# AcherStyx/SSD-Object-Detection

Hardware: AMD Instinct MI355X
Metric: images/sec SSD300 train step, batch 64 (higher is better)
Workload: dtype bf16; 1 GPU; BASELINE configs[2]: SSD300 full train step (anchor match+encode, image normalisation, conv fwd, loss, conv bwd, per-variable clip (64 variables) + Adam), per-GPU batch 64, 80 classes, synthetic COCO-shaped boxes; per_gpu_batch=64, global_batch=64, parallelism=single

## Files before the change

include/ssd_hip.h:

```cpp
#ifndef SSD_HIP_H
#define SSD_HIP_H

#include <stddef.h>
#include <stdint.h>

#ifdef __cplusplus
extern "C" {
#endif

typedef enum {
    SSD_OK = 0,
    SSD_ERR_ASSERT = -1,
    SSD_ERR_VALUE = -2,
    SSD_ERR_WORKSPACE = -3,
    SSD_ERR_LAUNCH = -4,
    SSD_ERR_UNSUPPORTED = -5
} ssd_status;

typedef enum { SSD_F32 = 0, SSD_BF16 = 1 } ssd_dtype;

int ssd_hip_abi_version(void);
const char* ssd_status_string(int status);

int ssd_priors_count(const int* grid_hw, int levels, const int* ratio_off);
// ... 189 lines not shown
int ssd_heads_bwd_data_sparse_levels(const ssd_head_grads* hg, const ssd_head_layers* hl, int B, unsigned level_mask,
                                     void* ws, size_t ws_bytes, void* stream);
size_t ssd_heads_bwd_weight_sparse_workspace_bytes(int B, const ssd_head_grads* hg, const ssd_head_layers* hl);
int ssd_heads_bwd_weight_sparse(const ssd_head_grads* hg, const ssd_head_layers* hl, int B, void* ws, size_t ws_bytes,
                                void* stream);

int ssd_head_grad_pack(const void* dloc, const void* dconf, void* out, int B, int hw, int per_cell, int classes,
                       int npad, int anchors_total, int level_off, void* stream);

int ssd_opt_block_elems(void);
int ssd_grad_clip_scales(const float* grad, long long n, const int32_t* tensor_block_off, int ntensors, float clip,
                         double* partial, float* scale, float* norms, void* stream);
int ssd_grad_apply_scale(float* grad, long long n, const int32_t* block_tensor, const float* scale, void* stream);
int ssd_grad_accumulate(float* acc, const float* grad, long long n, const int32_t* block_tensor, const float* scale,
                        int first, void* stream);
int ssd_adam_step(float* param, const float* grad, float* m, float* v, void* param_bf16, long long n,
                  const int32_t* block_tensor, const float* scale, float grad_scale, float lr_t, float beta1,
                  float beta2, float eps, void* stream);
int ssd_sgd_step(float* param, const float* grad, void* param_bf16, long long n, const int32_t* block_tensor,
                 const float* scale, float grad_scale, float lr, void* stream);

enum ssd_conv_plan {
    SSD_PLAN_KERNEL_MASK = 0xff,
    SSD_PLAN_C64B = 1, SSD_PLAN_P32_64, SSD_PLAN_P32_128, SSD_PLAN_8PH,
    SSD_PLAN_DMA_256_256, SSD_PLAN_DMA_256_128, SSD_PLAN_DMA_256_64, SSD_PLAN_DMA_128_64, SSD_PLAN_DMA_128_128,
    SSD_PLAN_CONV0_FWD, SSD_PLAN_P512, SSD_PLAN_PW,
    SSD_PLAN_WG_FIRST = 32, SSD_PLAN_WG_PATCH_16x16, SSD_PLAN_WG_PATCH_6x40, SSD_PLAN_WG_PATCH_10x24, SSD_PLAN_WG_TILE,
    SSD_PLAN_WG_GENERIC,
    SSD_PLAN_F_FLAT = 0x100,
    SSD_PLAN_F_ROWFLAT = 0x200,
    SSD_PLAN_F_SPLITK = 0x400,
    SSD_PLAN_F_POOL_FUSED = 0x800,
    SSD_PLAN_F_S2 = 0x1000,
    SSD_PLAN_F_REDUCE_WIDE = 0x2000
};
int ssd_conv2d_fwd_plan(int B, int H, int W, int Cin, int Cout, int ksize, int stride, int pad_t, int pad_l, int Ho, int Wo,
                        int pool, size_t ws_bytes);
int ssd_conv2d_head_fwd_plan(int B, int H, int W, int Cin, int per_cell, int classes, size_t ws_bytes);
int ssd_conv2d_bwd_data_plan(int B, int H, int W, int Cin, int Cout_pad, int ksize, int stride, int pad_t, int pad_l, int Ho,
                             int Wo, int accumulate, size_t ws_bytes);
int ssd_conv2d_bwd_weight_plan(int B, int H, int W, int Cin, int Cout, int ldy, int ksize, int stride, int pad_t, int pad_l,
                               int Ho, int Wo);
const char* ssd_conv_plan_name(int plan);
int ssd_conv2d_fwd_workgroups(int B, int H, int W, int Cin, int Cout, int ksize, int stride, int pad_t, int pad_l, int Ho,
                              int Wo, int pool, size_t ws_bytes);
int ssd_conv2d_bwd_data_workgroups(int B, int H, int W, int Cin, int Cout_pad, int ksize, int stride, int pad_t, int pad_l,
                                   int Ho, int Wo, int accumulate, size_t ws_bytes);

int ssd_dev_knob(const char* name, int value);

int ssd_dev_mfma_calibration_workgroups(void);
double ssd_dev_mfma_calibration_flops(int iters);
int ssd_dev_mfma_calibration(int iters, void* stamps, void* sink, void* stream);

#ifdef __cplusplus
}
#endif
#endif
```

ssd-object-detection_amd/_lib.py:

```python
import ctypes
import os

HERE = os.path.dirname(os.path.abspath(__file__))
LIB_PATH = os.path.join(HERE, os.environ.get("SSD_HIP_LIB", "libssd_hip.so"))

SSD_OK, SSD_ERR_ASSERT, SSD_ERR_VALUE, SSD_ERR_WORKSPACE, SSD_ERR_LAUNCH, SSD_ERR_UNSUPPORTED = 0, -1, -2, -3, -4, -5
SSD_MAX_LEVELS = 8

_c_int_p = ctypes.POINTER(ctypes.c_int)
_c_double_p = ctypes.POINTER(ctypes.c_double)
VP = ctypes.c_void_p


class PriorGrid(ctypes.Structure):
    _fields_ = [("levels", ctypes.c_int),
                ("grid_h", ctypes.c_int * SSD_MAX_LEVELS),
                ("grid_w", ctypes.c_int * SSD_MAX_LEVELS),
                ("per_cell", ctypes.c_int * SSD_MAX_LEVELS),
                ("verified", ctypes.c_int)]


class HeadGrads(ctypes.Structure):
    _fields_ = [("levels", ctypes.c_int),
                ("hw", ctypes.c_int * SSD_MAX_LEVELS),
# ... 88 lines not shown
    "ssd_conv2d_bwd_data_wgrad_first": (ctypes.c_int, [VP] * 6 + [ctypes.c_int] * 3 + [VP, ctypes.c_size_t, VP]),
    "ssd_conv2d_bwd_weight_workspace_bytes": (ctypes.c_size_t, [ctypes.c_int] * 7),
    "ssd_conv2d_bwd_weight": (ctypes.c_int, [VP, VP, VP, VP] + [ctypes.c_int] * 12 + [VP, ctypes.c_size_t, VP]),
    "ssd_weight_transpose": (ctypes.c_int, [VP, VP, ctypes.c_int, ctypes.c_int, ctypes.c_int, ctypes.c_int, VP]),
    "ssd_cast_bf16": (ctypes.c_int, [VP, VP, ctypes.c_longlong, VP]),
    "ssd_image_prep": (ctypes.c_int, [VP, VP, ctypes.c_int, ctypes.c_int, ctypes.c_int, ctypes.c_int, VP]),
    "ssd_image_resize_prep": (ctypes.c_int, [VP, VP, VP, VP, ctypes.c_int, ctypes.c_int, ctypes.c_int, VP]),
    "ssd_box_prep": (ctypes.c_int, [VP, VP, VP, VP, ctypes.c_int, ctypes.c_int, VP]),
    "ssd_augment_plan": (ctypes.c_int, [VP, VP, VP, VP, ctypes.c_int, ctypes.c_int, ctypes.c_int, ctypes.c_uint64,
                                        ctypes.c_int64, VP, VP, VP, VP, VP]),
    "ssd_augment_image": (ctypes.c_int, [VP, ctypes.c_int, VP, VP, VP, VP, ctypes.c_int, ctypes.c_int, ctypes.c_int, VP]),
    "ssd_maxpool2x2_fwd": (ctypes.c_int, [VP, VP] + [ctypes.c_int] * 6 + [VP]),
    "ssd_maxpool2x2_bwd": (ctypes.c_int, [VP, VP, VP, VP] + [ctypes.c_int] * 6 + [VP]),
    "ssd_weight_transpose_batched": (ctypes.c_int, [VP, ctypes.c_int, ctypes.c_int, VP]),
    "ssd_maxpool2x2_fwd_argmax": (ctypes.c_int, [VP, VP, VP] + [ctypes.c_int] * 6 + [VP]),
    "ssd_maxpool2x2_bwd_argmax": (ctypes.c_int, [VP, VP, VP] + [ctypes.c_int] * 6 + [VP]),
    "ssd_head_grad_pack": (ctypes.c_int, [VP, VP, VP] + [ctypes.c_int] * 7 + [VP]),
    "ssd_opt_block_elems": (ctypes.c_int, []),
    "ssd_grad_clip_scales": (ctypes.c_int, [VP, ctypes.c_longlong, VP, ctypes.c_int, ctypes.c_float, VP, VP, VP, VP]),
    "ssd_grad_apply_scale": (ctypes.c_int, [VP, ctypes.c_longlong, VP, VP, VP]),
    "ssd_grad_accumulate": (ctypes.c_int, [VP, VP, ctypes.c_longlong, VP, VP, ctypes.c_int, VP]),
    "ssd_adam_step": (ctypes.c_int, [VP, VP, VP, VP, VP, ctypes.c_longlong, VP, VP] + [ctypes.c_float] * 5 + [VP]),
    "ssd_sgd_step": (ctypes.c_int, [VP, VP, VP, ctypes.c_longlong, VP, VP, ctypes.c_float, ctypes.c_float, VP]),
    "ssd_dev_knob": (ctypes.c_int, [ctypes.c_char_p, ctypes.c_int]),
    "ssd_dev_mfma_calibration_workgroups": (ctypes.c_int, []),
    "ssd_dev_mfma_calibration_flops": (ctypes.c_double, [ctypes.c_int]),
    "ssd_dev_mfma_calibration": (ctypes.c_int, [ctypes.c_int, VP, VP, VP]),
    "ssd_conv2d_fwd_plan": (ctypes.c_int, [ctypes.c_int] * 12 + [ctypes.c_size_t]),
    "ssd_conv2d_head_fwd_plan": (ctypes.c_int, [ctypes.c_int] * 6 + [ctypes.c_size_t]),
    "ssd_conv2d_bwd_data_plan": (ctypes.c_int, [ctypes.c_int] * 12 + [ctypes.c_size_t]),
    "ssd_conv2d_fwd_workgroups": (ctypes.c_int, [ctypes.c_int] * 12 + [ctypes.c_size_t]),
    "ssd_conv2d_bwd_data_workgroups": (ctypes.c_int, [ctypes.c_int] * 12 + [ctypes.c_size_t]),
    "ssd_conv2d_bwd_weight_plan": (ctypes.c_int, [ctypes.c_int] * 12),
    "ssd_conv_plan_name": (ctypes.c_char_p, [ctypes.c_int]),
    "ssd_loss_workspace_bytes": (ctypes.c_size_t, [ctypes.c_int, ctypes.c_int, ctypes.c_int]),
    "ssd_loss_heads_workspace_bytes": (ctypes.c_size_t, [ctypes.c_int, ctypes.c_int, ctypes.c_int]),
    "ssd_loss_fwd_bwd_heads": (ctypes.c_int, [VP, VP, ctypes.c_int, VP, VP, VP, ctypes.c_int, ctypes.c_int, ctypes.c_int,
                                              ctypes.c_float, VP, _HG, VP, ctypes.c_size_t, ctypes.c_int, VP]),
    "ssd_heads_bwd_data_sparse_workspace_bytes": (ctypes.c_size_t, [ctypes.c_int, _HL]),
    "ssd_heads_bwd_data_sparse": (ctypes.c_int, [_HG, _HL, ctypes.c_int, VP, ctypes.c_size_t, VP]),
    "ssd_heads_bwd_data_sparse_levels": (ctypes.c_int, [_HG, _HL, ctypes.c_int, ctypes.c_uint, VP, ctypes.c_size_t, VP]),
    "ssd_heads_bwd_weight_sparse_workspace_bytes": (ctypes.c_size_t, [ctypes.c_int, _HG, _HL]),
    "ssd_heads_bwd_weight_sparse": (ctypes.c_int, [_HG, _HL, ctypes.c_int, VP, ctypes.c_size_t, VP]),
    "ssd_loss_fwd_bwd": (ctypes.c_int, [VP, VP, ctypes.c_int, VP, VP, VP, ctypes.c_int, ctypes.c_int, ctypes.c_int,
                                        ctypes.c_float, VP, VP, VP, VP, ctypes.c_size_t, VP]),
}

_lib = None


def lib():
    global _lib
    if _lib is None:
        if not os.path.exists(LIB_PATH):
            raise RuntimeError(
                "libssd_hip.so is missing (%s): build it with `python ssd-object-detection_amd/build.py` "
                "or __graft_entry__.build(); there is no CPU fallback." % LIB_PATH)
        try:
            import torch
        except ImportError:
            pass
        L = ctypes.CDLL(LIB_PATH)
        for name, (res, args) in _SIGNATURES.items():
            fn = getattr(L, name)
            fn.restype = res
            fn.argtypes = args
# ... 14 lines not shown
```

ssd-object-detection_amd/csrc/conv.hip:

```cpp
#include <atomic>
#include <climits>
#include <cstdint>
#include <cstring>
#include <type_traits>
#include "common.h"
#include <hip/hip_bf16.h>
#include <stdlib.h>

#include "conv_common.h"
namespace {

template <int EPI>
__global__ void k_igemm_finalize(ConvGeom g, Epilogue ep) {
    const int n4 = (g.N + 3) >> 2;
    const long long idx = (long long)blockIdx.x * blockDim.x + threadIdx.x;
    if (idx >= (long long)g.M * n4) return;
    const int m = (int)(idx / n4), n = (int)(idx - (long long)m * n4) * 4;
    const bool full = n + 3 < g.N;
    float v[4] = {0.f, 0.f, 0.f, 0.f};
    if (full && !(g.N & 3)) {
        for (int z = 0; z < ep.ksplit; ++z) {
            const float4 t = *reinterpret_cast<const float4*>(ep.slab + ((long long)z * g.M + m) * g.N + n);
            v[0] += t.x; v[1] += t.y; v[2] += t.z; v[3] += t.w;
        }
// ... 1678 lines not shown
                for (int c = 0; c < 4; ++c)
                    acc[a][c] = __builtin_amdgcn_mfma_f32_16x16x32_bf16(fa[a], fb[c], acc[a][c], 0, 0, 0);
                if constexpr (BIAS) accb[a] = __builtin_amdgcn_mfma_f32_16x16x32_bf16(fa[a], ones, accb[a], 0, 0, 0);
            }
        }
    };
    if (do_bias) run(std::true_type{}); else run(std::false_type{});

    float* out = slab_w + (long long)split * g.N * ktot;
#pragma unroll
    for (int a = 0; a < 8; ++a)
#pragma unroll
        for (int c = 0; c < 4; ++c) {
            const int col = col0 + wave_n * 64 + c * 16 + (lane & 15);
            if (col >= ktot) continue;
#pragma unroll
            for (int j = 0; j < 4; ++j) {
                const int co = co0 + wave_m * 128 + a * 16 + (lane >> 4) * 4 + j;
                if (co < g.N) out[(long long)co * ktot + col] = acc[a][c][j];
            }
        }
    if (do_bias && (lane & 15) == 0) {
        float* ob = slab_b + (long long)split * g.N;
#pragma unroll
        for (int a = 0; a < 8; ++a)
#pragma unroll
            for (int j = 0; j < 4; ++j) {
                const int co = co0 + wave_m * 128 + a * 16 + (lane >> 4) * 4 + j;
                if (co < g.N) ob[co] = accb[a][j];
            }
    }
}

template <int BH, int BW8>
struct WpGeom {
    static constexpr int BW = BW8 * 8;
    static constexpr int PW = BW + 2, PH = BH + 2;
    static constexpr int PPIX = PW * PH;
    static constexpr int P_INSTR = (PPIX * 8 + 63) / 64;
    static constexpr int P_BYTES = P_INSTR * 1024;
    static constexpr int NPG = (BH / 2) * BW8;
    static constexpr int KS = (NPG + 1) / 2;
    static constexpr int DY_PIX = KS * 32;
    static constexpr int DY_BYTES = DY_PIX * 128;
    static constexpr int DY_INSTR = DY_PIX / 8;
    static constexpr int BUF = DY_BYTES + P_BYTES;
    static_assert(BH % 2 == 0 && DY_INSTR % 8 == 0, "block shape");
};

__device__ __forceinline__ int wp_key(int px) { return (px >> 1) & 3; }

template <int BH, int BW8>
__global__ __launch_bounds__(512) void k_conv3x3_wgrad_patch(const bf16_raw* __restrict__ x, const bf16_raw* __restrict__ dy,
                                                             float* __restrict__ slab_w, float* __restrict__ slab_b,
                                                             ConvGeom g, int tiles_x, int tiles_y, int tiles_per_split,
                                                             int nsplit, int cout, int single_buf, int xg) {
    using G = WpGeom<BH, BW8>;
    extern __shared__ __attribute__((aligned(16))) char smem[];

    const int tid = threadIdx.x, lane = tid & 63;
    const int wave = __builtin_amdgcn_readfirstlane(tid >> 6);
    const int ct = wave & 3, role = wave >> 2;
    const int nchunk = g.C >> 6, cotiles = (cout + 63) >> 6;
    const int nunits = nchunk * cotiles * nsplit;
    const int j = blockIdx.x >> 3;
    int id = ((j / xg) * 8 + (blockIdx.x & 7)) * xg + j % xg;
    if (id >= nunits) return;
    const int chunk = id % nchunk; id /= nchunk;
    const int cot = id % cotiles;
    const int split = id / cotiles;
    const int co0 = cot * 64, ci0 = chunk * 64;
    const int ntiles = g.B * tiles_x * tiles_y;
    const int t_begin = split * tiles_per_split, t_end = min(ntiles, t_begin + tiles_per_split);

    const __amdgpu_buffer_rsrc_t xres = __builtin_amdgcn_make_buffer_rsrc((void*)x, 0, (unsigned)g.B * g.H * g.W * g.C * 2u, 0x00020000);
    const __amdgpu_buffer_rsrc_t dyres = __builtin_amdgcn_make_buffer_rsrc((void*)dy, 0, (unsigned)g.B * g.Ho * g.Wo * g.N * 2u, 0x00020000);
    constexpr unsigned WP_OOB = 0xfffffff0u;
    auto issue_dma = [&](int t, int buf) {
        int r = t;
        const int tx = r % tiles_x; r /= tiles_x;
        const int ty = r % tiles_y;
        const int b = r / tiles_y;
        const int y0 = ty * BH, x0 = tx * G::BW;
        char* base = smem + buf * G::BUF;
#pragma unroll
        for (int j = 0; j < G::DY_INSTR / 4; ++j) {
            const int i = ct + 4 * j;
            const int kk = 8 * i + (lane >> 3), sl = lane & 7;
            const int c16 = (((sl >> 1) ^ wp_key(kk)) << 1) | (sl & 1);
            const int pg = kk >> 4;
            const int rp = pg / BW8, xg = pg - rp * BW8;
            const int y = y0 + 2 * rp + ((kk >> 3) & 1), xx = x0 + xg * 8 + (kk & 7);
            const int co = co0 + c16 * 8;
            const bool ok = pg < G::NPG && y < g.Ho && xx < g.Wo && co < g.N;
            const unsigned off = ((unsigned)((b * g.Ho + y) * g.Wo + xx) * (unsigned)g.N + (unsigned)co) * 2u;
            __builtin_amdgcn_raw_ptr_buffer_load_lds(dyres, (lds_void*)(base + i * 1024), 16, ok ? off : WP_OOB, 0, 0, 0);
        }
#pragma unroll
        for (int j = 0; j < (G::P_INSTR + 3) / 4; ++j) {
            const int i = ct + 4 * j;
            if (i < G::P_INSTR) {
                const int pp = 8 * i + (lane >> 3), sl = lane & 7;
                const int c16 = (((sl >> 1) ^ wp_key(pp)) << 1) | (sl & 1);
                const int py = pp / G::PW, px = pp - py * G::PW;
                const int iy = y0 - 1 + py, ix = x0 - 1 + px;
                const bool ok = pp < G::PPIX && (unsigned)iy < (unsigned)g.H && (unsigned)ix < (unsigned)g.W;
                const unsigned off = ((unsigned)((b * g.H + iy) * g.W + ix) * (unsigned)g.C + (unsigned)(ci0 + c16 * 8)) * 2u;
                __builtin_amdgcn_raw_ptr_buffer_load_lds(xres, (lds_void*)(base + G::DY_BYTES + i * 1024), 16, ok ? off : WP_OOB, 0, 0, 0);
            }
        }
    };

    constexpr int LTAPS = 4;
    f32x4_t acc[4][9 - LTAPS];
    f32x4_t accb[4];
#pragma unroll
    for (int a = 0; a < 4; ++a) {
        accb[a] = f32x4_t{0.f, 0.f, 0.f, 0.f};
#pragma unroll
        for (int t5 = 0; t5 < 9 - LTAPS; ++t5) acc[a][t5] = f32x4_t{0.f, 0.f, 0.f, 0.f};
    }
    const bool do_bias = slab_b != nullptr && chunk == 0 && ct == 0 && role == 1;
    bf16x8_t ones;
#pragma unroll
    for (int i = 0; i < 8; ++i) ones[i] = (__bf16)1.0f;

    if (t_begin < t_end && role == 0) issue_dma(t_begin, 0);
    const int gq = lane >> 4, li = lane & 15;
    int abase[4];
    {
        const int kk0 = (gq >> 1) * 8 + (gq & 1) * 4 + (li >> 2);
#pragma unroll
        for (int a = 0; a < 4; ++a) abase[a] = kk0 * 128 + ((a ^ wp_key(kk0)) << 5) + (li & 3) * 8;
    }
    int gbase[8];
    {
        const int p0 = (gq >> 1) * G::PW + (gq & 1) * 4 + (li >> 2);
#pragma unroll
        for (int r = 0; r < 8; ++r) gbase[r] = G::DY_BYTES + (p0 + r) * 128 + ((ct ^ wp_key(p0 + r)) << 5) + (li & 3) * 8;
    }
    typedef __attribute__((address_space(3))) s16x4_t lds_s16x4;
    struct Frag { bf16x8_t fa[4]; bf16x8_t fb[9 - LTAPS]; };
    auto run = [&](auto role_tag, auto bias_tag) {
        constexpr int ROLE = decltype(role_tag)::value;
        constexpr bool BIAS = decltype(bias_tag)::value;
        constexpr int TAP0 = ROLE == 0 ? 0 : LTAPS, NTAP = ROLE == 0 ? LTAPS : 9 - LTAPS;
        auto load_frag = [&](Frag& f, const int (&ab)[4], const int (&gb)[8], auto ks_tag) {
            constexpr int ks = decltype(ks_tag)::value;
#pragma unroll
            for (int half = 0; half < 2; ++half)
#pragma unroll
                for (int a = 0; a < 4; ++a)
                    reinterpret_cast<s16x4_t*>(&f.fa[a])[half] =
                        lds_read_tr16_scoped(smem + ab[a] + (ks * 2 + half) * 2048, smem);
#pragma unroll
            for (int t5 = 0; t5 < NTAP; ++t5)
#pragma unroll
                for (int half = 0; half < 2; ++half) {
                    const int tap = TAP0 + t5;
                    const int pg = (ks * 2 + half) < G::NPG ? (ks * 2 + half) : 0;
                    const int rp = pg / BW8, xg = pg - rp * BW8;
                    const int ctap = (2 * rp + tap / 3) * G::PW + xg * 8 + (tap % 3);
                    reinterpret_cast<s16x4_t*>(&f.fb[t5])[half] =
                        lds_read_tr16_scoped(smem + gb[ctap & 7] + (ctap >> 3) * 1024, smem);
                }
        };
        for (int t = t_begin; t < t_end; ++t) {
            const int cur = (t - t_begin) & 1;
            asm volatile("s_waitcnt vmcnt(0)" ::: "memory");
            __syncthreads();
            if constexpr (ROLE == 0) { if (t + 1 < t_end) issue_dma(t + 1, cur ^ 1); }
            const int boff = cur * G::BUF;
            int ab[4], gb[8];
#pragma unroll
            for (int a = 0; a < 4; ++a) ab[a] = abase[a] + boff;
#pragma unroll
            for (int r = 0; r < 8; ++r) gb[r] = gbase[r] + boff;
            Frag f0, f1;
            auto mma = [&](const Frag& f) {
#pragma unroll
                for (int t5 = 0; t5 < NTAP; ++t5)
#pragma unroll
                    for (int a = 0; a < 4; ++a)
                        acc[a][t5] = __builtin_amdgcn_mfma_f32_16x16x32_bf16(f.fa[a], f.fb[t5], acc[a][t5], 0, 0, 0);
                if constexpr (BIAS) {
#pragma unroll
                    for (int a = 0; a < 4; ++a) accb[a] = __builtin_amdgcn_mfma_f32_16x16x32_bf16(f.fa[a], ones, accb[a], 0, 0, 0);
                }
            };
            auto weave = [&]() {
                constexpr int NR = 8 + 2 * NTAP, NM = 4 * NTAP;
// ... 452 lines not shown
    const int pix = (int)(r % hw);
    const int b = (int)(r / hw);
    const int n_loc = per_cell * 4, n_conf = per_cell * classes;
    const long long anchor0 = (long long)b * anchors_total + level_off + (long long)pix * per_cell;
    const bf16_raw* pl = dloc + anchor0 * 4;
    const bf16_raw* pc = dconf + anchor0 * classes - n_loc;
    if (!((per_cell | level_off | anchors_total) & 1)) {
        unsigned w4[4];
#pragma unroll
        for (int j = 0; j < 4; ++j) {
            const int n = ch * 8 + 2 * j;
            w4[j] = n < n_loc ? *reinterpret_cast<const unsigned*>(pl + n)
                              : (n < n_loc + n_conf ? *reinterpret_cast<const unsigned*>(pc + n) : 0u);
        }
        *reinterpret_cast<uint4*>(out + r * npad + ch * 8) = make_uint4(w4[0], w4[1], w4[2], w4[3]);
        return;
    }
    bf16_raw v[8];
#pragma unroll
    for (int j = 0; j < 8; ++j) {
        const int n = ch * 8 + j;
        v[j] = n < n_loc ? pl[n] : (n < n_loc + n_conf ? pc[n] : (bf16_raw)0);
    }
    *reinterpret_cast<uint4*>(out + r * npad + ch * 8) =
        make_uint4((unsigned)v[0] | ((unsigned)v[1] << 16), (unsigned)v[2] | ((unsigned)v[3] << 16),
                   (unsigned)v[4] | ((unsigned)v[5] << 16), (unsigned)v[6] | ((unsigned)v[7] << 16));
}

struct Knob { const char* name; std::atomic<int> value; };
constexpr int KNOB_UNSET = INT_MIN;
Knob g_knobs[] = {{"SSD_ABLATE", {KNOB_UNSET}}, {"SSD_DGRAD_S2", {KNOB_UNSET}}, 
                  {"SSD_CONV_PATCH", {KNOB_UNSET}}, {"SSD_CONV_TILE", {KNOB_UNSET}}, {"SSD_SPLITK", {KNOB_UNSET}},
                  {"SSD_WGRAD_PATCH", {KNOB_UNSET}},
                  {"SSD_WGRAD_PATCH_SHAPE", {KNOB_UNSET}}, {"SSD_WGRAD_TILE", {KNOB_UNSET}},
                  {"SSD_CONV_PATCH_FLAT", {KNOB_UNSET}}, {"SSD_WGRAD_FIRST", {KNOB_UNSET}}, {"SSD_CONV_FIRST", {KNOB_UNSET}},
                  {"SSD_WGRAD_PATCH_XCD", {KNOB_UNSET}}, {"SSD_CONV_C64", {KNOB_UNSET}}, {"SSD_CONV_POOL_FUSE", {KNOB_UNSET}},
                  {"SSD_CONV_PATCH_ROWFLAT", {KNOB_UNSET}}, {"SSD_MATCH_FUSED", {KNOB_UNSET}}, {"SSD_CONV_P512", {KNOB_UNSET}},
                  {"SSD_C64B_WGS", {KNOB_UNSET}}, {"SSD_CONV_PW", {KNOB_UNSET}}, {"SSD_PW_WGS", {KNOB_UNSET}},
                  {"SSD_SP_ABLATE", {KNOB_UNSET}}};
Knob* find_knob(const char* name) {
    for (Knob& k : g_knobs) if (!strcmp(k.name, name)) return &k;
    return nullptr;
}
int knob(const char* name, int dflt) {
    Knob* k = find_knob(name);
    if (!k) return dflt;
    const int v = k->value.load(std::memory_order_relaxed);
    return v == KNOB_UNSET ? dflt : v;
}

constexpr int PLAN_WANT_WGS = -1;
#define SSD_PLAN(ID_) do { if (plan) { if (*plan == PLAN_WANT_WGS) return SSD_ERR_UNSUPPORTED; *plan = (ID_); return SSD_OK; } } while (0)
#define SSD_PLAN_WGS(ID_, WGS_) do { if (plan) { *plan = *plan == PLAN_WANT_WGS ? (int)(WGS_) : (ID_); return SSD_OK; } } while (0)

template <int EPI>
bool staged_ok_host(const ConvGeom& g, const Epilogue& ep) {
    if (ep.slab) return false;
    if (EPI == EPI_HEAD) return true;
    return (g.N & 7) == 0 && (ep.ldo & 7) == 0;
}

template <int EPI>
int launch_igemm(const void* x, const void* w, const ConvGeom& g, const Epilogue& ep_in, hipStream_t s, void* ws = nullptr,
                 size_t ws_bytes = 0, bool* pooled = nullptr, int* plan = nullptr) {
    const bf16_raw* xp = static_cast<const bf16_raw*>(x);
    const bf16_raw* wp = static_cast<const bf16_raw*>(w);
    Epilogue ep = ep_in;
// ... 350 lines not shown
    static OnceLds set; if (ensure_lds(set, reinterpret_cast<const void*>(kern), (int)(C64B_W0_LDS)) != 0) return SSD_ERR_LAUNCH;
    hipLaunchKernelGGL(kern, dim3(grid), dim3(256), C64B_W0_LDS, s, static_cast<const bf16_raw*>(dy), static_cast<const bf16_raw*>(w_t),
                       g, ep, tiles_x, tiles_y, C64W0{static_cast<const bf16_raw*>(image), slab_w, dbias0 ? slab_b : nullptr});
    if (hipGetLastError() != hipSuccess) return SSD_ERR_LAUNCH;
    ssd_launch_wgrad_reduce(s, slab_w, 64ll * 72, 64ll * 72, dw0, slab_b, 64ll, 64, dbias0, (int)grid);
    return ssd_launch_status();
}

static bool wgrad_first_layer(int H, int W, int Ho, int Wo, int Cin, int Cout, int ldy, int ksize, int stride, int pad_t, int pad_l) {
    return knob("SSD_WGRAD_FIRST", 1) && Cin == 8 && Cout <= 64 && ldy <= 64 && ksize == 3 && stride == 1 && pad_t == 1 && pad_l == 1 &&
           H == Ho && W == Wo && H >= 16 && W >= 16;
}

static bool wgrad_use_patch(int H, int W, int Ho, int Wo, int Cin, int ksize, int stride, int pad_t, int pad_l) {
    const int mn = wgrad_patch_min_hw();
    return mn > 0 && ksize == 3 && stride == 1 && pad_t == 1 && pad_l == 1 && H == Ho && W == Wo && Cin % 64 == 0 &&
           H >= mn && W >= mn;
}

static int wgrad_patch_shape(int Ho, int Wo, int* bh, int* bw) {
    static const int shapes[3][3] = {{16, 16, 16}, {6, 40, 15}, {10, 24, 15}};
    int best = 0;
    double best_cost = 0;
    for (int i = 0; i < 3; ++i) {
        const double cost = (double)((Ho + shapes[i][0] - 1) / shapes[i][0]) * ((Wo + shapes[i][1] - 1) / shapes[i][1]);
        if (i == 0 || cost < best_cost) { best = i; best_cost = cost; }
    }
    const int forced = knob("SSD_WGRAD_PATCH_SHAPE", -1);
    if (forced >= 0 && forced < 3) best = forced;
    *bh = shapes[best][0]; *bw = shapes[best][1];
    return best;
}

static void wgrad_patch_plan(int B, int Ho, int Wo, int Cin, int Cout, int* tiles_x, int* tiles_y, int* tps, int* ns) {
    int bh, bw;
    wgrad_patch_shape(Ho, Wo, &bh, &bw);
    *tiles_x = (Wo + bw - 1) / bw; *tiles_y = (Ho + bh - 1) / bh;
    const int ntiles = B * *tiles_x * *tiles_y;
    const int groups = (Cin / 64) * ((Cout + 63) / 64);
    int want = 256 / groups;
    if (want < 1) want = 1;
    if (want > ntiles) want = ntiles;
    *tps = (ntiles + want - 1) / want;
    *ns = (ntiles + *tps - 1) / *tps;
}

constexpr int WG_BMO = 128, WG_BNC = 128;

static int wgrad_splits(long long M, int tiles) {
    long long want = 768 / tiles;
    long long maxs = (M + 511) / 512;
    if (want > maxs) want = maxs;
    if (want < 1) want = 1;
    if (want > 512) want = 512;
    return (int)want;
}

static bool wgrad_use_tile(long long M, int Cout, int ldy, long long ktot, long long x_elems) {
    return knob("SSD_WGRAD_TILE", 1) && Cout > 128 && ktot >= 256 && M >= 2048 && M * ldy < (1ll << 31) - 16 &&
           x_elems < (1ll << 31) - 16;
}

static int wgrad_tile_splits(long long M, int tiles, long long slab_elems) {
    int best = 1;
    double best_cost = 0;
    const long long maxs = M / 256 > 0 ? M / 256 : 1;
    for (int ns = 1; ns <= 64 && ns <= maxs; ++ns) {
        const long long rounds = ((long long)tiles * ns + 255) / 256;
        const long long steps = ((M + ns - 1) / ns + 63) / 64;
        const double cost = (double)rounds * steps * 2.2 + (double)ns * slab_elems * 8.0 / 4.0e6;
        if (ns == 1 || cost < best_cost) { best = ns; best_cost = cost; }
    }
    return best;
}

size_t ssd_conv2d_bwd_weight_workspace_bytes(int B, int Ho, int Wo, int Cin, int Cout, int ldy, int ksize) {
    if (B <= 0 || Ho <= 0 || Wo <= 0 || Cin <= 0 || Cout <= 0 || ldy < Cout || ksize <= 0) return 0;
// ... 16 lines not shown
        const int ns2 = wgrad_tile_splits((long long)B * Ho * Wo, t2, (long long)ldy * ktot);
        const size_t gen2 = (size_t)ns2 * ((size_t)ldy * ktot + ldy) * sizeof(float);
        if (gen2 > gen) gen = gen2;
    }
    return gen > patch_bytes ? gen : patch_bytes;
}

static int conv2d_bwd_weight_impl(const void* x, const void* dy, float* dw, float* dbias, int B, int H, int W, int Cin, int Cout,
                                  int ldy, int ksize, int stride, int pad_t, int pad_l, int Ho, int Wo, void* ws, size_t ws_bytes,
                                  void* stream, int* plan) {
    if (!x || !dy || !dw || !geom_ok(B, H, W, Cin, Ho, Wo, Cout, ksize) || stride <= 0 || ldy < Cout || ldy % 8) return SSD_ERR_VALUE;
    if (!ws || ws_bytes < ssd_conv2d_bwd_weight_workspace_bytes(B, Ho, Wo, Cin, Cout, ldy, ksize)) return SSD_ERR_WORKSPACE;
    ConvGeom g = make_geom(B, H, W, Cin, Ho, Wo, ldy, ksize, ksize, stride, 1, pad_t, pad_l);
    const long long ktot = g.ldw;
    if (wgrad_first_layer(H, W, Ho, Wo, Cin, Cout, ldy, ksize, stride, pad_t, pad_l)) {
        const int tx = (Wo + 15) / 16, ty = (Ho + 15) / 16, ntiles = B * tx * ty;
        const int ns = ntiles < 512 ? ntiles : 512;
        const int tps = (ntiles + ns - 1) / ns;
        SSD_PLAN(SSD_PLAN_WG_FIRST | ((ntiles + tps - 1) / tps >= 32 ? SSD_PLAN_F_REDUCE_WIDE : 0));
        float* slab_w = static_cast<float*>(ws);
        float* slab_b = slab_w + (size_t)ns * ldy * ktot;
        hipStream_t s = (hipStream_t)stream;
        static OnceLds set; if (ensure_lds(set, reinterpret_cast<const void*>(k_conv0_wgrad), (int)(2 * W0_BUF)) != 0) return SSD_ERR_LAUNCH;
        hipLaunchKernelGGL(k_conv0_wgrad, dim3((unsigned)((ntiles + tps - 1) / tps)), dim3(512), 2 * W0_BUF, s,
                           static_cast<const bf16_raw*>(x), static_cast<const bf16_raw*>(dy), slab_w, dbias ? slab_b : nullptr, g,
                           tx, ty, tps, Cout);
        if (hipGetLastError() != hipSuccess) return SSD_ERR_LAUNCH;
        const int nsr = (ntiles + tps - 1) / tps;
        ssd_launch_wgrad_reduce(s, slab_w, (long long)ldy * ktot, (long long)Cout * ktot, dw, slab_b, (long long)ldy, Cout, dbias, nsr);
        return ssd_launch_status();
    }
    if (wgrad_use_patch(H, W, Ho, Wo, Cin, ksize, stride, pad_t, pad_l) &&
        (long long)B * H * W * Cin * 2 < (1ll << 32) - 16 && (long long)B * Ho * Wo * ldy * 2 < (1ll << 32) - 16) {
        int tx, ty, tps, ns;
        wgrad_patch_plan(B, Ho, Wo, Cin, Cout, &tx, &ty, &tps, &ns);
        float* slab_w = static_cast<float*>(ws);
        float* slab_b = slab_w + (size_t)ns * ldy * ktot;
        hipStream_t s = (hipStream_t)stream;
        const int groups = (Cin / 64) * ((Cout + 63) / 64), nunits = groups * ns;
        int xg = 1;
        for (int d = groups; d >= 1; --d) {
            if (groups % d) continue;
            const int ngr = (nunits + d - 1) / d;
            const int load = ((ngr + 7) / 8) * d, fair = (nunits + 7) / 8;
            if (load * 100 <= fair * 107) { xg = d; break; }
        }
        if (!knob("SSD_WGRAD_PATCH_XCD", 1)) xg = 1;
        const unsigned grid = (unsigned)(8 * xg * ((nunits + 8 * xg - 1) / (8 * xg)));
        int bh, bw;
        const int shape = wgrad_patch_shape(Ho, Wo, &bh, &bw);
        SSD_PLAN((shape == 1 ? SSD_PLAN_WG_PATCH_6x40 : (shape == 2 ? SSD_PLAN_WG_PATCH_10x24 : SSD_PLAN_WG_PATCH_16x16)) |
                 (ns >= 32 ? SSD_PLAN_F_REDUCE_WIDE : 0));
#define SSD_LAUNCH_WP(BH_, BW8_)                                                                                    \
        do {                                                                                                        \
            using G_ = WpGeom<BH_, BW8_>;                                                                           \
            auto kern_ = k_conv3x3_wgrad_patch<BH_, BW8_>;                                                          \
            static OnceLds set_; if (ensure_lds(set_, reinterpret_cast<const void*>(kern_), (int)(2 * G_::BUF)) != 0) return SSD_ERR_LAUNCH; \
            hipLaunchKernelGGL(kern_, dim3(grid), dim3(512), (size_t)2 * G_::BUF, s,                                 \
                               static_cast<const bf16_raw*>(x), static_cast<const bf16_raw*>(dy), slab_w,          \
                               dbias ? slab_b : nullptr, g, tx, ty, tps, ns, Cout, 0, xg);                          \
        } while (0)
        if (shape == 1) SSD_LAUNCH_WP(6, 5);
        else if (shape == 2) SSD_LAUNCH_WP(10, 3);
        else SSD_LAUNCH_WP(16, 2);
#undef SSD_LAUNCH_WP
        if (hipGetLastError() != hipSuccess) return SSD_ERR_LAUNCH;
        ssd_launch_wgrad_reduce(s, slab_w, (long long)ldy * ktot, (long long)Cout * ktot, dw, slab_b, (long long)ldy, Cout, dbias, ns);
        return ssd_launch_status();
    }
    if (wgrad_use_tile(g.M, Cout, ldy, ktot, (long long)B * H * W * Cin)) {
        const int ctiles = (int)((ktot + 255) / 256), mtiles = (Cout + 255) / 256;
        const int ns = wgrad_tile_splits(g.M, ctiles * mtiles, (long long)ldy * ktot);
        int mps = (int)(((long long)g.M + ns - 1) / ns);
        mps = (mps + 63) / 64 * 64;
        SSD_PLAN(SSD_PLAN_WG_TILE | (ns >= 32 ? SSD_PLAN_F_REDUCE_WIDE : 0));
        float* slab_w = static_cast<float*>(ws);
        float* slab_b = slab_w + (size_t)ns * ldy * ktot;
        hipStream_t s = (hipStream_t)stream;
        static OnceLds set; if (ensure_lds(set, reinterpret_cast<const void*>(k_conv_wgrad_tile), (int)(4 * WT_TILE)) != 0) return SSD_ERR_LAUNCH;
        hipLaunchKernelGGL(k_conv_wgrad_tile, dim3(ctiles * mtiles * ns), dim3(512), 4 * WT_TILE, s,
                           static_cast<const bf16_raw*>(x), static_cast<const bf16_raw*>(dy), slab_w, dbias ? slab_b : nullptr, g,
                           mps, ns, Cout);
        if (hipGetLastError() != hipSuccess) return SSD_ERR_LAUNCH;
        ssd_launch_wgrad_reduce(s, slab_w, (long long)ldy * ktot, (long long)Cout * ktot, dw, slab_b, (long long)ldy, Cout, dbias, ns);
        return ssd_launch_status();
    }
    const int ctiles = (int)((ktot + WG_BNC - 1) / WG_BNC), mtiles = (Cout + WG_BMO - 1) / WG_BMO;
    const int ns = wgrad_splits(g.M, ctiles * mtiles);
    int mps = (int)(((long long)g.M + ns - 1) / ns);
    mps = (mps + 63) / 64 * 64;
    SSD_PLAN(SSD_PLAN_WG_GENERIC | (ns >= 32 ? SSD_PLAN_F_REDUCE_WIDE : 0));
    float* slab_w = static_cast<float*>(ws);
    float* slab_b = slab_w + (size_t)ns * ldy * ktot;
    hipStream_t s = (hipStream_t)stream;
    const bf16_raw* xp = static_cast<const bf16_raw*>(x);
    const bf16_raw* dyp = static_cast<const bf16_raw*>(dy);
    float* sb = dbias ? slab_b : nullptr;
// ... 104 lines not shown
int ssd_conv2d_fwd_workgroups(int B, int H, int W, int Cin, int Cout, int ksize, int stride, int pad_t, int pad_l, int Ho, int Wo,
                              int pool, size_t ws_bytes) {
    int plan = PLAN_WANT_WGS, rc;
    void* ws = ws_bytes ? PLAN_PTR : nullptr;
    if (pool) {
        const int Hp = (Ho + 1) / 2, Wp = (Wo + 1) / 2;
        rc = conv2d_fwd_pool_impl(PLAN_PTR, PLAN_PTR, nullptr, pool == 2 ? nullptr : PLAN_PTR, PLAN_PTR, PLAN_PTR, B, H, W, Cin, Cout,
                                  ksize, stride, pad_t, pad_l, Ho, Wo, 1, Hp, Wp, ws, ws_bytes, nullptr, &plan);
    } else {
        rc = conv2d_fwd_impl(PLAN_PTR, PLAN_PTR, nullptr, PLAN_PTR, B, H, W, Cin, Cout, ksize, stride, pad_t, pad_l, Ho, Wo, 1, ws,
                             ws_bytes, nullptr, &plan);
    }
    return rc != SSD_OK ? rc : plan;
}

int ssd_conv2d_bwd_data_workgroups(int B, int H, int W, int Cin, int Cout_pad, int ksize, int stride, int pad_t, int pad_l, int Ho,
                                   int Wo, int accumulate, size_t ws_bytes) {
    int plan = PLAN_WANT_WGS;
    const int rc = conv2d_bwd_data_impl(PLAN_PTR, PLAN_PTR, nullptr, PLAN_PTR, B, H, W, Cin, Cout_pad, ksize, stride, pad_t, pad_l,
                                        Ho, Wo, accumulate, ws_bytes ? PLAN_PTR : nullptr, ws_bytes, nullptr, &plan);
    return rc != SSD_OK ? rc : plan;
}

int ssd_conv2d_bwd_weight_plan(int B, int H, int W, int Cin, int Cout, int ldy, int ksize, int stride, int pad_t, int pad_l,
                               int Ho, int Wo) {
    int plan = 0;
    const size_t need = ssd_conv2d_bwd_weight_workspace_bytes(B, Ho, Wo, Cin, Cout, ldy, ksize);
    const int rc = conv2d_bwd_weight_impl(PLAN_PTR, PLAN_PTR, reinterpret_cast<float*>(PLAN_PTR), reinterpret_cast<float*>(PLAN_PTR),
                                          B, H, W, Cin, Cout, ldy, ksize, stride, pad_t, pad_l, Ho, Wo, PLAN_PTR, need, nullptr,
                                          &plan);
    return rc != SSD_OK ? rc : plan;
}

const char* ssd_conv_plan_name(int plan) {
    switch (plan & SSD_PLAN_KERNEL_MASK) {
        case SSD_PLAN_C64B: return "k_conv3x3_c64b";
        case SSD_PLAN_P32_64: return "k_conv3x3_patch32<64>";
        case SSD_PLAN_P32_128: return "k_conv3x3_patch32<128>";
        case SSD_PLAN_P512: return "k_conv3x3_p512";
        case SSD_PLAN_8PH: return "k_conv_igemm_8ph";
        case SSD_PLAN_PW: return "k_pw_gemm";
        case SSD_PLAN_DMA_256_256: return "k_conv_igemm_dma<256,256>";
        case SSD_PLAN_DMA_256_128: return "k_conv_igemm_dma<256,128>";
        case SSD_PLAN_DMA_256_64: return "k_conv_igemm_dma<256,64>";
        case SSD_PLAN_DMA_128_64: return "k_conv_igemm_dma<128,64>";
        case SSD_PLAN_DMA_128_128: return "k_conv_igemm_dma<128,128>";
        case SSD_PLAN_CONV0_FWD: return "k_conv0_fwd";
        case SSD_PLAN_WG_FIRST: return "k_conv0_wgrad";
        case SSD_PLAN_WG_PATCH_16x16: return "k_conv3x3_wgrad_patch<16,2>";
        case SSD_PLAN_WG_PATCH_6x40: return "k_conv3x3_wgrad_patch<6,5>";
        case SSD_PLAN_WG_PATCH_10x24: return "k_conv3x3_wgrad_patch<10,3>";
        case SSD_PLAN_WG_TILE: return "k_conv_wgrad_tile";
        case SSD_PLAN_WG_GENERIC: return "k_conv_wgrad";
        default: return "?";
    }
}

int ssd_weight_transpose(const void* w, void* w_t, int Cout, int ksize, int Cin, int Cout_pad, void* stream) {
    if (!w || !w_t || Cout <= 0 || ksize <= 0 || Cin <= 0 || Cout_pad < Cout || Cout_pad % 8) return SSD_ERR_VALUE;
    const long long total = (long long)Cin * ksize * ksize * Cout_pad;
    hipLaunchKernelGGL(k_weight_transpose, dim3((unsigned)((total + 255) / 256)), dim3(256), 0, (hipStream_t)stream,
                       static_cast<const bf16_raw*>(w), static_cast<bf16_raw*>(w_t), Cout, ksize, ksize, Cin, Cout_pad);
    return ssd_launch_status();
}

int ssd_weight_transpose_batched(const long long* desc, int ntensors, int max_tiles, void* stream) {
// ... 77 lines not shown
```

Baseline: 7259 images/sec.

## Tile 3x3 wgrad patch kernel over padded position or row strips across images

Adds two tiling modes to the 3x3 weight-gradient patch kernel. Instead of fixed 2D tiles per image, work is cut into linear strips of padded output positions (or padded row strips) that span image boundaries, with the padding acting as a halo. The goal is to cut the wasted partial tiles at image edges and the total tile count for odd feature-map sizes. It uses mul-hi reciprocal division for index decoding and adds extra template variants. The mode is chosen by a heuristic and is on by default through a new knob.

```diff
diff --git a/include/ssd_hip.h b/include/ssd_hip.h
--- a/include/ssd_hip.h
+++ b/include/ssd_hip.h
@@ -245,7 +245,9 @@
     SSD_PLAN_F_SPLITK = 0x400,
     SSD_PLAN_F_POOL_FUSED = 0x800,
     SSD_PLAN_F_S2 = 0x1000,
-    SSD_PLAN_F_REDUCE_WIDE = 0x2000
+    SSD_PLAN_F_REDUCE_WIDE = 0x2000,
+    SSD_PLAN_F_WG_POS_STRIPS = 0x4000,
+    SSD_PLAN_F_WG_ROW_STRIPS = 0x8000
 };
 int ssd_conv2d_fwd_plan(int B, int H, int W, int Cin, int Cout, int ksize, int stride, int pad_t, int pad_l, int Ho, int Wo,
                         int pool, size_t ws_bytes);
@@ -259,6 +261,8 @@
                               int Wo, int pool, size_t ws_bytes);
 int ssd_conv2d_bwd_data_workgroups(int B, int H, int W, int Cin, int Cout_pad, int ksize, int stride, int pad_t, int pad_l,
                                    int Ho, int Wo, int accumulate, size_t ws_bytes);
+int ssd_conv2d_bwd_weight_blocks(int B, int H, int W, int Cin, int Cout, int ldy, int ksize, int stride, int pad_t, int pad_l,
+                                 int Ho, int Wo);
 
 int ssd_dev_knob(const char* name, int value);
 
diff --git a/ssd-object-detection_amd/_lib.py b/ssd-object-detection_amd/_lib.py
--- a/ssd-object-detection_amd/_lib.py
+++ b/ssd-object-detection_amd/_lib.py
@@ -144,6 +144,7 @@
     "ssd_conv2d_fwd_workgroups": (ctypes.c_int, [ctypes.c_int] * 12 + [ctypes.c_size_t]),
     "ssd_conv2d_bwd_data_workgroups": (ctypes.c_int, [ctypes.c_int] * 12 + [ctypes.c_size_t]),
     "ssd_conv2d_bwd_weight_plan": (ctypes.c_int, [ctypes.c_int] * 12),
+    "ssd_conv2d_bwd_weight_blocks": (ctypes.c_int, [ctypes.c_int] * 12),
     "ssd_conv_plan_name": (ctypes.c_char_p, [ctypes.c_int]),
     "ssd_loss_workspace_bytes": (ctypes.c_size_t, [ctypes.c_int, ctypes.c_int, ctypes.c_int]),
     "ssd_loss_heads_workspace_bytes": (ctypes.c_size_t, [ctypes.c_int, ctypes.c_int, ctypes.c_int]),
diff --git a/ssd-object-detection_amd/csrc/conv.hip b/ssd-object-detection_amd/csrc/conv.hip
--- a/ssd-object-detection_amd/csrc/conv.hip
+++ b/ssd-object-detection_amd/csrc/conv.hip
@@ -1734,6 +1734,8 @@
     }
 }
 
+enum { WP_IMAGE = 0, WP_POS = 1, WP_ROWS = 2 };
+
 template <int BH, int BW8>
 struct WpGeom {
     static constexpr int BW = BW8 * 8;
@@ -1752,11 +1754,23 @@
 
 __device__ __forceinline__ int wp_key(int px) { return (px >> 1) & 3; }
 
-template <int BH, int BW8>
+__device__ __forceinline__ unsigned wp_div(unsigned n, unsigned m) { return __umulhi(n, m); }
+
+__device__ __forceinline__ unsigned wp_pos_offset(int p, int B, int H, int W, int ld, int cb, bool inside, unsigned mw,
+                                                  unsigned mh, unsigned oob) {
+    const unsigned up = (unsigned)p;
+    const unsigned R = wp_div(up, mw), c = up - R * ((unsigned)W + 1u);
+    const unsigned b = wp_div(R, mh), y = R - b * ((unsigned)H + 1u);
+    const bool ok = inside && c != 0u && y < (unsigned)H && b < (unsigned)B;
+    const unsigned off = (((b * (unsigned)H + y) * (unsigned)W + (c - 1u)) * (unsigned)ld + (unsigned)cb) * 2u;
+    return ok ? off : oob;
+}
+
+template <int BH, int BW8, int STRIP>
 __global__ __launch_bounds__(512) void k_conv3x3_wgrad_patch(const bf16_raw* __restrict__ x, const bf16_raw* __restrict__ dy,
                                                              float* __restrict__ slab_w, float* __restrict__ slab_b,
                                                              ConvGeom g, int tiles_x, int tiles_y, int tiles_per_split,
-                                                             int nsplit, int cout, int single_buf, int xg) {
+                                                             int nsplit, int cout, int ntiles, int xg, unsigned mw, unsigned mh) {
     using G = WpGeom<BH, BW8>;
     extern __shared__ __attribute__((aligned(16))) char smem[];
 
@@ -1772,19 +1786,43 @@
     const int cot = id % cotiles;
     const int split = id / cotiles;
     const int co0 = cot * 64, ci0 = chunk * 64;
-    const int ntiles = g.B * tiles_x * tiles_y;
     const int t_begin = split * tiles_per_split, t_end = min(ntiles, t_begin + tiles_per_split);
 
     const __amdgpu_buffer_rsrc_t xres = __builtin_amdgcn_make_buffer_rsrc((void*)x, 0, (unsigned)g.B * g.H * g.W * g.C * 2u, 0x00020000);
     const __amdgpu_buffer_rsrc_t dyres = __builtin_amdgcn_make_buffer_rsrc((void*)dy, 0, (unsigned)g.B * g.Ho * g.Wo * g.N * 2u, 0x00020000);
     constexpr unsigned WP_OOB = 0xfffffff0u;
     auto issue_dma = [&](int t, int buf) {
+        char* base = smem + buf * G::BUF;
+        if constexpr (STRIP == WP_POS) {
+            const int p0 = t * 256;
+#pragma unroll
+            for (int j = 0; j < G::DY_INSTR / 4; ++j) {
+                const int i = ct + 4 * j;
+                const int kk = 8 * i + (lane >> 3), sl = lane & 7;
+                const int c16 = (((sl >> 1) ^ wp_key(kk)) << 1) | (sl & 1);
+                const int co = co0 + c16 * 8;
+                __builtin_amdgcn_raw_ptr_buffer_load_lds(dyres, (lds_void*)(base + i * 1024), 16,
+                                                         wp_pos_offset(p0 + kk, g.B, g.H, g.W, g.N, co, co < g.N, mw, mh, WP_OOB), 0, 0, 0);
+            }
+            const int plen = 256 + 2 * (g.W + 2);
+#pragma unroll
+            for (int j = 0; j < (G::P_INSTR + 3) / 4; ++j) {
+                const int i = ct + 4 * j;
+                if (i < G::P_INSTR) {
+                    const int pp = 8 * i + (lane >> 3), sl = lane & 7;
+                    const int c16 = (((sl >> 1) ^ wp_key(pp)) << 1) | (sl & 1);
+                    const int p = p0 - (g.W + 2) + pp;
+                    __builtin_amdgcn_raw_ptr_buffer_load_lds(xres, (lds_void*)(base + G::DY_BYTES + i * 1024), 16,
+                                                             wp_pos_offset(p, g.B, g.H, g.W, g.C, ci0 + c16 * 8, p >= 0 && pp < plen, mw, mh, WP_OOB), 0, 0, 0);
+                }
+            }
+            return;
+        }
         int r = t;
         const int tx = r % tiles_x; r /= tiles_x;
-        const int ty = r % tiles_y;
-        const int b = r / tiles_y;
-        const int y0 = ty * BH, x0 = tx * G::BW;
-        char* base = smem + buf * G::BUF;
+        const int ty = STRIP == WP_ROWS ? r : r % tiles_y;
+        const int b0 = STRIP == WP_ROWS ? (ty * BH) / (g.H + 1) : r / tiles_y;
+        const int y0 = STRIP == WP_ROWS ? ty * BH - b0 * (g.H + 1) : ty * BH, x0 = tx * G::BW;
 #pragma unroll
         for (int j = 0; j < G::DY_INSTR / 4; ++j) {
             const int i = ct + 4 * j;
@@ -1792,9 +1830,11 @@
             const int c16 = (((sl >> 1) ^ wp_key(kk)) << 1) | (sl & 1);
             const int pg = kk >> 4;
             const int rp = pg / BW8, xg = pg - rp * BW8;
-            const int y = y0 + 2 * rp + ((kk >> 3) & 1), xx = x0 + xg * 8 + (kk & 7);
+            int y = y0 + 2 * rp + ((kk >> 3) & 1), b = b0;
+            const int xx = x0 + xg * 8 + (kk & 7);
+            if constexpr (STRIP == WP_ROWS) { const bool nxt = y > g.Ho; y = nxt ? y - (g.Ho + 1) : y; b = nxt ? b + 1 : b; }
             const int co = co0 + c16 * 8;
-            const bool ok = pg < G::NPG && y < g.Ho && xx < g.Wo && co < g.N;
+            const bool ok = pg < G::NPG && y < g.Ho && xx < g.Wo && co < g.N && (STRIP != WP_ROWS || b < g.B);
             const unsigned off = ((unsigned)((b * g.Ho + y) * g.Wo + xx) * (unsigned)g.N + (unsigned)co) * 2u;
             __builtin_amdgcn_raw_ptr_buffer_load_lds(dyres, (lds_void*)(base + i * 1024), 16, ok ? off : WP_OOB, 0, 0, 0);
         }
@@ -1805,8 +1845,10 @@
                 const int pp = 8 * i + (lane >> 3), sl = lane & 7;
                 const int c16 = (((sl >> 1) ^ wp_key(pp)) << 1) | (sl & 1);
                 const int py = pp / G::PW, px = pp - py * G::PW;
-                const int iy = y0 - 1 + py, ix = x0 - 1 + px;
-                const bool ok = pp < G::PPIX && (unsigned)iy < (unsigned)g.H && (unsigned)ix < (unsigned)g.W;
+                int iy = y0 - 1 + py, b = b0;
+                const int ix = x0 - 1 + px;
+                if constexpr (STRIP == WP_ROWS) { const bool nxt = iy > g.H; iy = nxt ? iy - (g.H + 1) : iy; b = nxt ? b + 1 : b; }
+                const bool ok = pp < G::PPIX && (unsigned)iy < (unsigned)g.H && (unsigned)ix < (unsigned)g.W && (STRIP != WP_ROWS || b < g.B);
                 const unsigned off = ((unsigned)((b * g.H + iy) * g.W + ix) * (unsigned)g.C + (unsigned)(ci0 + c16 * 8)) * 2u;
                 __builtin_amdgcn_raw_ptr_buffer_load_lds(xres, (lds_void*)(base + G::DY_BYTES + i * 1024), 16, ok ? off : WP_OOB, 0, 0, 0);
             }
@@ -1836,7 +1878,15 @@
         for (int a = 0; a < 4; ++a) abase[a] = kk0 * 128 + ((a ^ wp_key(kk0)) << 5) + (li & 3) * 8;
     }
     int gbase[8];
-    {
+    if constexpr (STRIP == WP_POS) {
+        const int kk0 = gq * 4 + (li >> 2);
+#pragma unroll
+        for (int r = 0; r < 8; ++r) {
+            const int tap = role * LTAPS + r;
+            const int q = kk0 + (tap / 3) * (g.W + 1) + tap % 3;
+            gbase[r] = G::DY_BYTES + q * 128 + ((ct ^ wp_key(q)) << 5) + (li & 3) * 8;
+        }
+    } else {
         const int p0 = (gq >> 1) * G::PW + (gq & 1) * 4 + (li >> 2);
 #pragma unroll
         for (int r = 0; r < 8; ++r) gbase[r] = G::DY_BYTES + (p0 + r) * 128 + ((ct ^ wp_key(p0 + r)) << 5) + (li & 3) * 8;
@@ -1859,6 +1909,11 @@
             for (int t5 = 0; t5 < NTAP; ++t5)
 #pragma unroll
                 for (int half = 0; half < 2; ++half) {
+                    if constexpr (STRIP == WP_POS) {
+                        reinterpret_cast<s16x4_t*>(&f.fb[t5])[half] =
+                            lds_read_tr16_scoped(smem + gb[t5] + (ks * 2 + half) * 2048, smem);
+                        continue;
+                    }
                     const int tap = TAP0 + t5;
                     const int pg = (ks * 2 + half) < G::NPG ? (ks * 2 + half) : 0;
                     const int rp = pg / BW8, xg = pg - rp * BW8;
@@ -2377,7 +2432,7 @@
 Knob g_knobs[] = {{"SSD_ABLATE", {KNOB_UNSET}}, {"SSD_DGRAD_S2", {KNOB_UNSET}}, 
                   {"SSD_CONV_PATCH", {KNOB_UNSET}}, {"SSD_CONV_TILE", {KNOB_UNSET}}, {"SSD_SPLITK", {KNOB_UNSET}},
                   {"SSD_WGRAD_PATCH", {KNOB_UNSET}},
-                  {"SSD_WGRAD_PATCH_SHAPE", {KNOB_UNSET}}, {"SSD_WGRAD_TILE", {KNOB_UNSET}},
+                  {"SSD_WGRAD_PATCH_SHAPE", {KNOB_UNSET}}, {"SSD_WGRAD_PATCH_STRIP", {KNOB_UNSET}}, {"SSD_WGRAD_TILE", {KNOB_UNSET}},
                   {"SSD_CONV_PATCH_FLAT", {KNOB_UNSET}}, {"SSD_WGRAD_FIRST", {KNOB_UNSET}}, {"SSD_CONV_FIRST", {KNOB_UNSET}},
                   {"SSD_WGRAD_PATCH_XCD", {KNOB_UNSET}}, {"SSD_CONV_C64", {KNOB_UNSET}}, {"SSD_CONV_POOL_FUSE", {KNOB_UNSET}},
                   {"SSD_CONV_PATCH_ROWFLAT", {KNOB_UNSET}}, {"SSD_MATCH_FUSED", {KNOB_UNSET}}, {"SSD_CONV_P512", {KNOB_UNSET}},
@@ -2794,17 +2849,30 @@
     return best;
 }
 
-static void wgrad_patch_plan(int B, int Ho, int Wo, int Cin, int Cout, int* tiles_x, int* tiles_y, int* tps, int* ns) {
+static int wgrad_patch_plan(int B, int Ho, int Wo, int Cin, int Cout, int* tiles_x, int* tiles_y, int* tps, int* ns,
+                            int* ntiles_out = nullptr) {
     int bh, bw;
     wgrad_patch_shape(Ho, Wo, &bh, &bw);
     *tiles_x = (Wo + bw - 1) / bw; *tiles_y = (Ho + bh - 1) / bh;
-    const int ntiles = B * *tiles_x * *tiles_y;
+    int ntiles = B * *tiles_x * *tiles_y, strip = WP_IMAGE;
+    if (knob("SSD_WGRAD_PATCH_STRIP", 1)) {
+        const long long npos = (long long)B * (Ho + 1) * (Wo + 1), nrows = (long long)B * (Ho + 1);
+        const long long pos_blocks = (npos + 255) / 256, row_blocks = (nrows + bh - 1) / bh * *tiles_x;
+        if (256 + 2 * (Wo + 2) <= (bh + 2) * (bw + 2) && pos_blocks < ntiles &&
+            (npos + 1024) * ((Ho > Wo ? Ho : Wo) + 1) < (1ll << 32)) {
+            strip = WP_POS; ntiles = (int)pos_blocks;
+        } else if (Ho >= bh && row_blocks < ntiles) {
+            strip = WP_ROWS; ntiles = (int)row_blocks; *tiles_y = (int)((nrows + bh - 1) / bh);
+        }
+    }
+    if (ntiles_out) *ntiles_out = ntiles;
     const int groups = (Cin / 64) * ((Cout + 63) / 64);
     int want = 256 / groups;
     if (want < 1) want = 1;
     if (want > ntiles) want = ntiles;
     *tps = (ntiles + want - 1) / want;
     *ns = (ntiles + *tps - 1) / *tps;
+    return strip;
 }
 
 constexpr int WG_BMO = 128, WG_BNC = 128;
@@ -2887,8 +2955,8 @@
     }
     if (wgrad_use_patch(H, W, Ho, Wo, Cin, ksize, stride, pad_t, pad_l) &&
         (long long)B * H * W * Cin * 2 < (1ll << 32) - 16 && (long long)B * Ho * Wo * ldy * 2 < (1ll << 32) - 16) {
-        int tx, ty, tps, ns;
-        wgrad_patch_plan(B, Ho, Wo, Cin, Cout, &tx, &ty, &tps, &ns);
+        int tx, ty, tps, ns, ntiles;
+        const int strip = wgrad_patch_plan(B, Ho, Wo, Cin, Cout, &tx, &ty, &tps, &ns, &ntiles);
         float* slab_w = static_cast<float*>(ws);
         float* slab_b = slab_w + (size_t)ns * ldy * ktot;
         hipStream_t s = (hipStream_t)stream;
@@ -2904,20 +2972,29 @@
         const unsigned grid = (unsigned)(8 * xg * ((nunits + 8 * xg - 1) / (8 * xg)));
         int bh, bw;
         const int shape = wgrad_patch_shape(Ho, Wo, &bh, &bw);
-        SSD_PLAN((shape == 1 ? SSD_PLAN_WG_PATCH_6x40 : (shape == 2 ? SSD_PLAN_WG_PATCH_10x24 : SSD_PLAN_WG_PATCH_16x16)) |
-                 (ns >= 32 ? SSD_PLAN_F_REDUCE_WIDE : 0));
-#define SSD_LAUNCH_WP(BH_, BW8_)                                                                                    \
+        SSD_PLAN_WGS((shape == 1 ? SSD_PLAN_WG_PATCH_6x40 : (shape == 2 ? SSD_PLAN_WG_PATCH_10x24 : SSD_PLAN_WG_PATCH_16x16)) |
+                     (strip == WP_POS ? SSD_PLAN_F_WG_POS_STRIPS : (strip == WP_ROWS ? SSD_PLAN_F_WG_ROW_STRIPS : 0)) |
+                     (ns >= 32 ? SSD_PLAN_F_REDUCE_WIDE : 0), ntiles);
+        const unsigned mw = (unsigned)((1ull << 32) / (unsigned)(Wo + 1)) + 1u, mh = (unsigned)((1ull << 32) / (unsigned)(Ho + 1)) + 1u;
+#define SSD_LAUNCH_WP(BH_, BW8_, STRIP_)                                                                            \
         do {                                                                                                        \
             using G_ = WpGeom<BH_, BW8_>;                                                                           \
-            auto kern_ = k_conv3x3_wgrad_patch<BH_, BW8_>;                                                          \
+            auto kern_ = k_conv3x3_wgrad_patch<BH_, BW8_, STRIP_>;                                                  \
             static OnceLds set_; if (ensure_lds(set_, reinterpret_cast<const void*>(kern_), (int)(2 * G_::BUF)) != 0) return SSD_ERR_LAUNCH; \
             hipLaunchKernelGGL(kern_, dim3(grid), dim3(512), (size_t)2 * G_::BUF, s,                                 \
                                static_cast<const bf16_raw*>(x), static_cast<const bf16_raw*>(dy), slab_w,          \
-                               dbias ? slab_b : nullptr, g, tx, ty, tps, ns, Cout, 0, xg);                          \
+                               dbias ? slab_b : nullptr, g, tx, ty, tps, ns, Cout, ntiles, xg, mw, mh);             \
         } while (0)
-        if (shape == 1) SSD_LAUNCH_WP(6, 5);
-        else if (shape == 2) SSD_LAUNCH_WP(10, 3);
-        else SSD_LAUNCH_WP(16, 2);
+#define SSD_LAUNCH_WP_STRIP(BH_, BW8_)                                                                              \
+        do {                                                                                                        \
+            if (strip == WP_POS) SSD_LAUNCH_WP(BH_, BW8_, WP_POS);                                                  \
+            else if (strip == WP_ROWS) SSD_LAUNCH_WP(BH_, BW8_, WP_ROWS);                                           \
+            else SSD_LAUNCH_WP(BH_, BW8_, WP_IMAGE);                                                                \
+        } while (0)
+        if (shape == 1) SSD_LAUNCH_WP_STRIP(6, 5);
+        else if (shape == 2) SSD_LAUNCH_WP_STRIP(10, 3);
+        else SSD_LAUNCH_WP_STRIP(16, 2);
+#undef SSD_LAUNCH_WP_STRIP
 #undef SSD_LAUNCH_WP
         if (hipGetLastError() != hipSuccess) return SSD_ERR_LAUNCH;
         ssd_launch_wgrad_reduce(s, slab_w, (long long)ldy * ktot, (long long)Cout * ktot, dw, slab_b, (long long)ldy, Cout, dbias, ns);
@@ -3088,6 +3165,16 @@
     return rc != SSD_OK ? rc : plan;
 }
 
+int ssd_conv2d_bwd_weight_blocks(int B, int H, int W, int Cin, int Cout, int ldy, int ksize, int stride, int pad_t, int pad_l,
+                                 int Ho, int Wo) {
+    int plan = PLAN_WANT_WGS;
+    const size_t need = ssd_conv2d_bwd_weight_workspace_bytes(B, Ho, Wo, Cin, Cout, ldy, ksize);
+    const int rc = conv2d_bwd_weight_impl(PLAN_PTR, PLAN_PTR, reinterpret_cast<float*>(PLAN_PTR), reinterpret_cast<float*>(PLAN_PTR),
+                                          B, H, W, Cin, Cout, ldy, ksize, stride, pad_t, pad_l, Ho, Wo, PLAN_PTR, need, nullptr,
+                                          &plan);
+    return rc != SSD_OK ? rc : plan;
+}
+
 const char* ssd_conv_plan_name(int plan) {
     switch (plan & SSD_PLAN_KERNEL_MASK) {
         case SSD_PLAN_C64B: return "k_conv3x3_c64b";
```

Result: no change. 7258 images/sec (-0.0%).
